# davidbau/rewriting

Measured on AMD Instinct MI355X. Metric: images/sec StyleGANv2-1024 fwd, higher is better.
Workload: dtype f32 (conv operands split into exact f16 pairs from 32x32 up, f32 accumulate); 1 GPU; stylegan2-1024 generator forward (FFHQ-1024 architecture); batch_per_gpu=64, mconv=seq, weights=synthetic seed 0, parallelism=seeds partitioned per rank, no collective, matrix_mode=split, direct_sums=auto

## Files before the change

### include/rewriting_hip.h

```cpp
#ifndef REWRITING_HIP_H
#define REWRITING_HIP_H

#include <stdint.h>

#ifdef __cplusplus
extern "C" {
#endif

typedef void* rw_stream_t;

#define RW_ERR_BAD_ARGUMENT 10001
#define RW_ERR_UNSUPPORTED  10002

int rw_abi_version(void);
const char* rw_error_string(int code);


int rw_fused_bias_act_f32(const float* x, const float* b, const float* ref, float* y,
                          int64_t n, int64_t step_b, int64_t size_b,
                          int act, int grad, float alpha, float scale, rw_stream_t stream);
int rw_fused_bias_act_f16(const uint16_t* x, const uint16_t* b, const uint16_t* ref, uint16_t* y,
                          int64_t n, int64_t step_b, int64_t size_b,
                          int act, int grad, float alpha, float scale, rw_stream_t stream);
int rw_fused_bias_act_f64(const double* x, const double* b, const double* ref, double* y,
// ... 146 lines not shown
                                           const float* post_scale, float u_inv, const float* x_amax,
                                           float* y_amax, rw_stream_t stream);

int rw_dconv3x3_supported(int out_ch, int in_ch, int h, int w);
long long rw_packed_dconv_weight_elems(int out_ch, int in_ch);
int rw_pack_dconv_weight_f32(const float* w, float* wp, int out_ch, int in_ch, float u_scale, rw_stream_t stream);
int rw_dconv3x3_f32(const float* x, const float* wp, float* y, int batch, int in_ch, int out_ch, int h, int w,
                    float w_scale, const rw_conv_epilogue* ep, float u_inv, const float* x_amax, float* y_amax,
                    rw_stream_t stream);
int rw_dconv3x3_rgb_partials(int out_ch);
int rw_dconv3x3_rgb_partial_f32(const float* x, const float* wp, float* y, int batch, int in_ch, int out_ch, int h, int w,
                                float w_scale, const rw_conv_epilogue* ep, const rw_rgb_epilogue* rgb, float u_inv,
                                const float* x_amax, float* y_amax, rw_stream_t stream);
int rw_rgb_combine_f32(const float* partials, int n_part, const float* bias, const float* skip, float* y, int batch,
                       int64_t hw, rw_stream_t stream);
int rw_rgb_combine_up_f32(const float* partials, int n_part, const float* bias, const float* skip_half, const float* k4,
                          float* y, int batch, int h, int w, rw_stream_t stream);
int rw_dconv3x3_to_rgb_supported(int out_ch, int in_ch, int h, int w);
int rw_dconv3x3_to_rgb_f32(const float* x, const float* wp, int batch, int in_ch, int out_ch, int h, int w,
                           float w_scale, const rw_conv_epilogue* ep, const rw_rgb_epilogue* rgb, float u_inv,
                           const float* x_amax, rw_stream_t stream);
int rw_dconv_transpose_blur_supported(int out_ch, int in_ch, int h, int w);
long long rw_packed_dconv_transpose_blur_weight_elems(int out_ch, int in_ch);
int rw_pack_dconv_transpose_blur_weight_f32(const float* w, const float* k4, float* wp, int out_ch, int in_ch,
                                            float u_scale, rw_stream_t stream);
int rw_dconv_transpose3x3s2_blur_f32(const float* x, const float* wp, float* y, int batch, int in_ch, int out_ch, int h,
                                     int w, float w_scale, const rw_conv_epilogue* ep, const float* post_scale,
                                     float u_inv, const float* x_amax, float* y_amax, rw_stream_t stream);

int rw_tconv_blur_supported(int out_ch, int in_ch, int h, int w);
int rw_tconv_blur_f32(const float* x, const float* wp, const float* k4, float* y, int batch, int in_ch, int out_ch, int h,
                      int w, float w_scale, const rw_conv_epilogue* ep, const float* post_scale, float u_inv,
                      const float* x_amax, float* y_amax, rw_stream_t stream);

int rw_conv_transpose3x3s2_winoh_supported(int out_ch, int in_ch, int h, int w);
long long rw_packed_conv_transpose_winoh_elems(int out_ch, int in_ch);
int rw_pack_conv_transpose_winoh_f32(const float* w, float* uf, int out_ch, int in_ch, float u_scale, rw_stream_t stream);
int rw_conv_transpose3x3s2_winoh_f32(const float* x, const float* uf, float* y, int batch, int in_ch, int out_ch,
                                     int h, int w, float w_scale, const float* style, const float* demod, float u_inv,
                                     const float* x_amax, rw_stream_t stream);

int rw_noise_add_f32(const float* x, const float* noise, const float* noise_w, float* y,
                     int batch, int channels, int64_t hw, rw_stream_t stream);

int rw_blur_noise_act_f32(const float* x, const float* k4, const float* noise, const float* noise_w,
                          const float* bias, float* y, int batch, int channels, int out_h, int out_w,
                          rw_stream_t stream);
int rw_blur_noise_act_scaled_f32(const float* x, const float* k4, const float* noise, const float* noise_w,
                                 const float* bias, const float* post_scale, float* y, int batch, int channels,
                                 int out_h, int out_w, rw_stream_t stream);
int rw_blur_noise_act_amax_f32(const float* x, const float* k4, const float* noise, const float* noise_w,
                               const float* bias, const float* post_scale, float* y, int batch, int channels,
                               int out_h, int out_w, float* y_amax, rw_stream_t stream);

int rw_to_rgb_f32(const float* x, const float* w, const float* style, const float* bias,
                  const float* skip, float* y, int batch, int in_ch, int64_t hw, float w_scale,
                  rw_stream_t stream);


int64_t rw_second_moment_workspace_bytes(int channels, int64_t rows);
int rw_second_moment_f32(const float* a, float* mom2, int64_t rows, int channels, int64_t hw,
                         int layout, void* workspace, rw_stream_t stream);

int rw_channel_sums_f32(const float* a, float* sums, int64_t rows, int channels, int64_t hw,
                        int layout, int square_input, rw_stream_t stream);

// ... 153 lines not shown
```

### rewriting_amd/_lib.py

```python
import ctypes
import os
from ctypes import (POINTER, Structure, c_char_p, c_double, c_float, c_int, c_int32, c_int64, c_uint,
                    c_void_p)

_HERE = os.path.dirname(os.path.abspath(__file__))
LIB_PATH = os.environ.get('RW_HIP_LIB') or os.path.join(_HERE, 'librewriting_hip.so')

ABI_VERSION = 11


class ConvEpilogue(Structure):
    _fields_ = [('style', c_void_p), ('demod', c_void_p), ('noise', c_void_p),
                ('noise_w', c_void_p), ('bias', c_void_p), ('act', c_int)]


class RgbEpilogue(Structure):
    _fields_ = [('weight', c_void_p), ('style', c_void_p), ('bias', c_void_p), ('skip', c_void_p),
                ('out', c_void_p), ('scale', c_float)]


LPIPS_MAX_TAPS = 8


class LpipsMaps(Structure):
# ... 121 lines not shown
    'rw_conv_transpose3x3s2_blur_wino4h_f32': (c_int, [c_void_p, c_void_p, c_void_p, c_int, c_int, c_int, c_int,
                                                       c_int, c_float, POINTER(ConvEpilogue), c_void_p, c_float,
                                                       c_void_p, c_void_p, c_void_p]),
    'rw_dconv3x3_supported': (c_int, [c_int, c_int, c_int, c_int]),
    'rw_packed_dconv_weight_elems': (ctypes.c_longlong, [c_int, c_int]),
    'rw_pack_dconv_weight_f32': (c_int, [c_void_p, c_void_p, c_int, c_int, c_float, c_void_p]),
    'rw_dconv3x3_f32': (c_int, [c_void_p, c_void_p, c_void_p, c_int, c_int, c_int, c_int, c_int, c_float,
                                POINTER(ConvEpilogue), c_float, c_void_p, c_void_p, c_void_p]),
    'rw_dconv3x3_rgb_partials': (c_int, [c_int]),
    'rw_dconv3x3_rgb_partial_f32': (c_int, [c_void_p, c_void_p, c_void_p, c_int, c_int, c_int, c_int, c_int, c_float,
                                            POINTER(ConvEpilogue), POINTER(RgbEpilogue), c_float, c_void_p, c_void_p,
                                            c_void_p]),
    'rw_rgb_combine_f32': (c_int, [c_void_p, c_int, c_void_p, c_void_p, c_void_p, c_int, c_int64, c_void_p]),
    'rw_rgb_combine_up_f32': (c_int, [c_void_p, c_int, c_void_p, c_void_p, c_void_p, c_void_p, c_int, c_int, c_int,
                                      c_void_p]),
    'rw_conv3x3_wino4_to_rgb_up_f32': (c_int, [c_void_p, c_void_p, c_int, c_int, c_int, c_int, c_int, c_float,
                                               POINTER(ConvEpilogue), POINTER(RgbEpilogue), c_void_p, c_void_p,
                                               c_void_p]),
    'rw_conv3x3_wino4h_to_rgb_up_f32': (c_int, [c_void_p, c_void_p, c_int, c_int, c_int, c_int, c_int, c_float,
                                                POINTER(ConvEpilogue), POINTER(RgbEpilogue), c_float, c_void_p, c_void_p,
                                                c_void_p, c_void_p]),
    'rw_dconv3x3_to_rgb_supported': (c_int, [c_int, c_int, c_int, c_int]),
    'rw_dconv3x3_to_rgb_f32': (c_int, [c_void_p, c_void_p, c_int, c_int, c_int, c_int, c_int, c_float,
                                       POINTER(ConvEpilogue), POINTER(RgbEpilogue), c_float, c_void_p, c_void_p]),
    'rw_dconv_transpose_blur_supported': (c_int, [c_int, c_int, c_int, c_int]),
    'rw_packed_dconv_transpose_blur_weight_elems': (ctypes.c_longlong, [c_int, c_int]),
    'rw_pack_dconv_transpose_blur_weight_f32': (c_int, [c_void_p, c_void_p, c_void_p, c_int, c_int, c_float, c_void_p]),
    'rw_dconv_transpose3x3s2_blur_f32': (c_int, [c_void_p, c_void_p, c_void_p, c_int, c_int, c_int, c_int, c_int,
                                                 c_float, POINTER(ConvEpilogue), c_void_p, c_float, c_void_p, c_void_p,
                                                 c_void_p]),
    'rw_tconv_blur_supported': (c_int, [c_int, c_int, c_int, c_int]),
    'rw_tconv_blur_f32': (c_int, [c_void_p, c_void_p, c_void_p, c_void_p, c_int, c_int, c_int, c_int, c_int, c_float,
                                  POINTER(ConvEpilogue), c_void_p, c_float, c_void_p, c_void_p, c_void_p]),
    'rw_conv_transpose_blur_wino4_supported': (c_int, [c_int, c_int, c_int, c_int]),
    'rw_packed_conv_transpose_blur_wino4_elems': (ctypes.c_longlong, [c_int, c_int]),
    'rw_pack_conv_transpose_blur_weight_wino4_f32': (c_int, [c_void_p, c_void_p, c_void_p, c_int, c_int, c_void_p]),
    'rw_conv_transpose3x3s2_blur_wino4_f32': (c_int, [c_void_p, c_void_p, c_void_p, c_int, c_int, c_int, c_int,
                                                      c_int, c_float, POINTER(ConvEpilogue), c_void_p, c_void_p]),
    'rw_blur_noise_act_scaled_f32': (c_int, [c_void_p, c_void_p, c_void_p, c_void_p, c_void_p, c_void_p, c_void_p,
                                             c_int, c_int, c_int, c_int, c_void_p]),
    'rw_blur_noise_act_amax_f32': (c_int, [c_void_p, c_void_p, c_void_p, c_void_p, c_void_p, c_void_p, c_void_p,
                                           c_int, c_int, c_int, c_int, c_void_p, c_void_p]),
    'rw_solve_ksplit': (c_int, [c_int, c_int, c_int, c_int]),
    'rw_solve_supported': (c_int, [c_int] * 7),
    'rw_solve_scratch_elems': (c_int, [c_int] * 5 + [POINTER(ctypes.c_longlong)]),
    'rw_solve_step_f32': (c_int, [POINTER(SolveProblem), c_int, c_void_p]),
    'rw_solve_run_supported': (c_int, [c_int] * 7),
    'rw_solve_run_scratch_elems': (ctypes.c_longlong, [c_int] * 5),
    'rw_solve_run_f32': (c_int, [POINTER(SolveProblem), c_int, c_int, c_int, c_int, c_int, c_void_p, c_void_p]),
    'rw_project_weight_f32': (c_int, [c_void_p, c_void_p, c_void_p, c_void_p, c_int, c_int, c_int,
                                      c_int, c_float, c_void_p]),
    'rw_conv_wgrad_ksplit': (c_int, [c_int] * 6),
    'rw_conv_wgrad_f32': (c_int, [c_void_p] * 6 + [c_int] * 6 + [c_float, c_void_p]),
    'rw_rowdot_f32': (c_int, [c_void_p, c_void_p, c_void_p, ctypes.c_longlong, ctypes.c_longlong, c_void_p]),
    'rw_to_rgb_input_grad_f32': (c_int, [c_void_p, c_void_p, c_void_p, c_void_p, c_int, c_int, c_int64, c_float,
                                         c_void_p]),
    'rw_to_rgb_weight_sums_scratch_elems': (ctypes.c_longlong, [c_int, c_int, c_int64]),
    'rw_to_rgb_weight_sums_f32': (c_int, [c_void_p, c_void_p, c_void_p, c_void_p, c_int, c_int, c_int64, c_void_p]),
    'rw_bias_relu_pool_f32': (c_int, [c_void_p, c_void_p, c_void_p, c_void_p, c_int, c_int, c_int, c_int, c_void_p]),
    'rw_bias_relu_pool_grad_f32': (c_int, [c_void_p, c_void_p, c_void_p, c_int, c_int, c_int, c_int, c_int, c_void_p]),
    'rw_conv3x3_rgb_f32': (c_int, [c_void_p, c_void_p, c_void_p, c_void_p, c_int, c_int, c_int, c_int, c_void_p]),
    'rw_conv3x3_rgb_input_grad_f32': (c_int, [c_void_p, c_void_p, c_void_p, c_int, c_int, c_int, c_int, c_void_p]),
    'rw_lpips_tap_f32': (c_int, [c_void_p, c_void_p, c_void_p, c_void_p, c_int, c_int, c_int, c_int64, c_void_p]),
    'rw_lpips_reduce_scratch_elems': (ctypes.c_longlong, [c_int, c_int64]),
    'rw_lpips_combine_f32': (c_int, [POINTER(LpipsMaps), c_void_p, c_void_p, c_void_p, c_int, c_void_p, c_void_p, c_void_p,
                                     c_int, c_int, c_int, c_void_p]),
# ... 58 lines not shown
```

### rewriting_amd/csrc/rw_tconv.hip

```cpp
#include "rw_common.h"
#include <stdio.h>

struct TconvProblem {
  const float* x; const unsigned char* wp; float* y; const float* k4;
  const float* style; const float* demod; const float* noise; const float* noise_w; const float* bias; int act;
  const float* post;
  int batch, in_ch, out_ch, h, w;
  int tiles_x, tiles_y, o_tiles;
  float w_scale, u_inv;
  const float* x_amax; float* y_amax;
};

#define TC_TX 32
#define TC_PC (TC_TX + 2)
#define TC_WC (TC_TX + 3)
#define TC_ZP 72
#define TC_WCH 9216

#ifndef TC_LDS_PAD
#define TC_LDS_PAD 0
#endif
#ifndef TC_ITEM_G
#define TC_ITEM_G 1
#endif
#ifndef TC_AHEAD
#define TC_AHEAD 1
#endif
#ifndef TC_STAGE_PRIO
#define TC_STAGE_PRIO 0
#endif
#ifndef TC_ABL
#define TC_ABL 0
#endif

__device__ __forceinline__ rw_f16x8 tc_pair_hq(rw_f32x2 h, rw_f16x8 q) {
  const rw_f32x4 qq = __builtin_bit_cast(rw_f32x4, q);
  const rw_f32x4 d = {h[0], h[1], qq[0], qq[1]};
  return __builtin_bit_cast(rw_f16x8, d);
}
#ifndef TC_PROF
#define TC_PROF 0
#endif
#if TC_PROF
__device__ unsigned long long tc_prof[64];
extern "C" int rw_tconv_prof(unsigned long long* out) {
  return (int)hipMemcpyFromSymbol(out, HIP_SYMBOL(tc_prof), sizeof(unsigned long long) * 64);
}
#define TP_DECL(...) unsigned long long __VA_ARGS__
#define TP_NOW(t) t = (unsigned long long)clock64()
#define TP_ADD(var, t) { const unsigned long long tp_n = (unsigned long long)clock64(); var += tp_n - t; t = tp_n; }
#else
#define TP_DECL(...)
#define TP_NOW(t)
#define TP_ADD(var, t)
#endif
__device__ __forceinline__ float tc_mul(float a, float b) {
  float r;
  asm("v_mul_f32 %0, %1, %2" : "=v"(r) : "v"(a), "v"(b));
  return r;
}

template <int TY, int WAVES, int NT>
__device__ __forceinline__ void tconv_body(const TconvProblem& p) {
  constexpr int THREADS = 64 * WAVES;
  constexpr int PR = TY + 2;
  constexpr int NPOS = PR * TC_PC, NBLK = (NPOS + 15) / 16, BPW = (NBLK + WAVES - 1) / WAVES;
  constexpr int WR = TY + 3, NPIX = WR * TC_WC;
  constexpr int BUFB = NPIX * 64;
  constexpr int ZR = 2 * PR, CHS = ZR * TC_ZP + 4;
  static_assert(8 * CHS * 4 <= 2 * BUFB, "the z tile of eight channels fits the window buffers");
  constexpr int SR = 2 * TY * 128 / THREADS;
  static_assert(WAVES % 4 == 0 && THREADS % 128 == 0 && SR * (THREADS / 128) == 2 * TY && (SR == 4 || SR == 8),
                "four or eight output rows per strip segment");
  constexpr int OC = 16 * NT, WCH = NT * TC_WCH;
  __shared__ __attribute__((aligned(16))) unsigned char Ls[2 * BUFB];
  __shared__ __attribute__((aligned(16))) unsigned char Wl[2 * WCH];
  __shared__ __attribute__((aligned(16))) float St[512];
  __shared__ float Sc[OC], Bs[OC], Po[OC], Kf[16], Red[WAVES];
#if TC_LDS_PAD
  constexpr int PADB = TY == 16 ? 163840 - 2 * BUFB - 2 * WCH - 2048 - 4 * 64 - 4 * WAVES - 64 : 16;
  __shared__ unsigned char Pad[PADB];
  if (p.batch < 0) Pad[threadIdx.x] = 1;
#endif

  const int tid = threadIdx.x, lane = tid & 63;
  const int wave = __builtin_amdgcn_readfirstlane(tid >> 6);
  const int lk = lane >> 4, lt = lane & 15;

  int ot, tx, ty, ib;
  rw_tile_digits(p, rw_xcd_remap(blockIdx.x, gridDim.x), ot, tx, ty, ib);
  const int I0 = ty * TY, J0 = tx * TC_TX;
  const int64_t hw = (int64_t)p.h * p.w;
  const int NC = p.in_ch >> 4, T = 9 * NC;

  float in_scale, out_scale;
  {
    const float smax = rw_block_max<WAVES>(rw_style_absmax_wave<64 * WAVES>(p, ib, tid), lane, wave, Red);
    rw_split_scales<14>(rw_bound_load(p.x_amax) * smax, p.u_inv, in_scale, out_scale);
  }
  const float gain = p.act ? 1.4142135623730951f : 1.f, slope = p.act ? 0.2f : 1.f;
  for (int i = tid; i < p.in_ch; i += THREADS) St[i] = (p.style ? p.style[(int64_t)ib * p.in_ch + i] : 1.0f) * in_scale;
  if (tid < OC) {
    const int o = OC * ot + tid;
    Sc[tid] = (p.demod ? p.demod[(int64_t)ib * p.out_ch + o] * p.w_scale : p.w_scale) * out_scale * gain;
    Bs[tid] = p.act ? p.bias[o] * gain : 0.f;
    Po[tid] = p.post ? p.post[(int64_t)ib * p.out_ch + o] : 1.f;
  }
  if (tid < 16) {
    const int a = tid >> 2, c = tid & 3;
    Kf[tid] = p.k4[(3 - a) * 4 + (3 - c)];
  }
  const float noise_wg = p.noise ? p.noise_w[0] * gain : 0.f;
  __syncthreads();

  constexpr int NSL = WAVES / 4;
  const int g = wave & 3, hsel = wave >> 2;
  const __amdgpu_buffer_rsrc_t xsrc = rw_image_rsrc(p.x, ib, p.in_ch, hw);
  const int hw4 = (int)hw * 4;
  constexpr int IPR = TC_TX / 4 + 2, NITEM = WR * IPR;
  constexpr int SI = (NITEM + 64 * NSL - 1) / (64 * NSL), LPP = ((NITEM + SI * NSL - 1) / (SI * NSL) + 3) & ~3;
  static_assert(SI <= 2 && LPP <= 64 && LPP * SI * NSL >= NITEM, "one or two pieces per wave cover the window");
  int xoff[SI], lofa[SI], lofb[SI], lok[SI];
#pragma unroll
  for (int s = 0; s < SI; ++s) {
    const int li = TC_ITEM_G == 4 ? (lane & 3) * (LPP / 4) + (lane >> 2) : lane;
    const int it = LPP * (NSL * s + hsel) + li;
    const bool mine = lane < LPP && it < NITEM;
    const int r = it / IPR, j = it - r * IPR;
    const int iy = I0 - 2 + r, ix = J0 - 4 + 4 * j;
    const bool ok = mine && iy >= 0 && iy < p.h && ix >= 0 && ix < p.w;
    xoff[s] = ok ? (iy * p.w + ix) * 4 : 0x7ffffff0;
    const int cc0 = 4 * j - 2;
    lofa[s] = (r * TC_WC + cc0) * 64 + ((g ^ rw_swz(cc0 & 0x7ffffffe)) << 4);
    lofb[s] = (r * TC_WC + cc0 + 2) * 64 + ((g ^ rw_swz(cc0 + 2)) << 4);
// ... 14 lines not shown
  };
  auto stage_store_part = [&](int c, int buf, auto s_tag, auto e0_tag, auto e1_tag) __attribute__((always_inline)) {
    constexpr int s = decltype(s_tag)::value, E0 = decltype(e0_tag)::value, E1 = decltype(e1_tag)::value;
    const rw_f32x4 sv = *reinterpret_cast<const rw_f32x4*>(&St[16 * c + 4 * g]);
    unsigned char* dst = Ls + buf * BUFB;
#pragma unroll
    for (int e = E0; e < E1; ++e) {
      const float v0 = tc_mul(raw[s][0][e], sv[0]), v1 = tc_mul(raw[s][1][e], sv[1]), v2 = tc_mul(raw[s][2][e], sv[2]),
                  v3 = tc_mul(raw[s][3][e], sv[3]);
      rw_f16x8 word = rw_split4(v0, v1, v2, v3);
      if (TC_ABL & 256)
        word = __builtin_bit_cast(rw_f16x8, rw_f32x4{raw[s][0][e], raw[s][1][e], raw[s][2][e], raw[s][3][e]});
      if (TC_ABL & 512) { asm volatile("" :: "v"(word)); }
      else if (lok[s] & (1 << e)) *reinterpret_cast<rw_f16x8*>(dst + (e < 2 ? lofa[s] : lofb[s]) + (e & 1) * 64) = word;
    }
  };
  const unsigned char* wsrc = p.wp + (int64_t)(NT * ot) * T * 1024;
  constexpr int NPC = NT * (TC_WCH / 16), NWP = (NPC + THREADS - 1) / THREADS;
  rw_f32x4 wraw[NWP];
  auto wstage_load = [&](int c) __attribute__((always_inline)) {
#pragma unroll
    for (int k = 0; k < NWP; ++k) {
      const int pc = tid + k * THREADS < NPC ? tid + k * THREADS : NPC - 1;
      const int n = pc / (TC_WCH / 16), r = pc - n * (TC_WCH / 16);
      wraw[k] = *reinterpret_cast<const rw_f32x4*>(wsrc + ((int64_t)n * T + 9 * c) * 1024 + r * 16);
    }
  };
  auto wstage_store = [&](int buf) __attribute__((always_inline)) {
    unsigned char* dst = Wl + buf * WCH;
#pragma unroll
    for (int k = 0; k < NWP; ++k)
      if ((k + 1) * THREADS <= NPC || tid + k * THREADS < NPC)
        *reinterpret_cast<rw_f32x4*>(dst + (tid + k * THREADS) * 16) = wraw[k];
  };

  unsigned pb0[BPW], pb1[BPW];
#pragma unroll
  for (int b = 0; b < BPW; ++b) {
    int q = 16 * (wave + WAVES * b) + lt;
    q = q < NPOS ? q : NPOS - 1;
    const int r = q / TC_PC, c = q - r * TC_PC;
    pb0[b] = (unsigned)((r * TC_WC + c + 1) * 64 + ((lk ^ rw_swz(c + 1)) << 4));
    pb1[b] = (unsigned)((r * TC_WC + c) * 64 + ((lk ^ rw_swz(c)) << 4));
  }

  rw_f32x4 acc[BPW][NT][4];
#pragma unroll
  for (int b = 0; b < BPW; ++b)
#pragma unroll
    for (int n = 0; n < NT; ++n)
#pragma unroll
      for (int ph = 0; ph < 4; ++ph) acc[b][n][ph] = rw_f32x4{0.f, 0.f, 0.f, 0.f};

#define TB_MFMA(PH, A, B) acc[b][n][PH] = __builtin_amdgcn_mfma_f32_16x16x32_f16(A, B, acc[b][n][PH], 0, 0, 0)
#define TB_UH(T_) rw_expand(*reinterpret_cast<const rw_f32x2*>(wb + n * TC_WCH + (T_) * 1024))
#define TB_UL(T_) (*reinterpret_cast<const rw_f32x2*>(wb + n * TC_WCH + (T_) * 1024 + 512))
#define TC_PIX(OFF) (*reinterpret_cast<const rw_f16x8*>(lb + (OFF)))
#define TC_VH(OFF) (*reinterpret_cast<const rw_f32x2*>(lb + (OFF)))
#define TC_MFMA(PH, A, B) acc[b][PH] = __builtin_amdgcn_mfma_f32_16x16x32_f16(A, B, acc[b][PH], 0, 0, 0)
#define TC_UH(T_) rw_expand(*reinterpret_cast<const rw_f32x2*>(wb + (T_) * 1024))
#define TC_UL(T_) (*reinterpret_cast<const rw_f32x2*>(wb + (T_) * 1024 + 512))
  TP_DECL(tp = 0, tp_all = 0, tp_g0 = 0, tp_s0 = 0, tp_g1 = 0, tp_g2 = 0, tp_s1 = 0, tp_bar = 0, tp_pro = 0);
  auto chunk = [&](int c, auto last_tag) __attribute__((always_inline)) {
    constexpr bool LAST = decltype(last_tag)::value != 0;
    const int buf = c & 1;
    const unsigned char* lb = Ls;
    const unsigned char* wb = Wl + buf * WCH + lane * 8;
    TP_NOW(tp);
    constexpr bool st = !LAST;
    const int c2 = c + 2 < NC ? c + 2 : NC - 1;
    auto hook = [&](auto grp_tag, int b) __attribute__((always_inline)) {
      constexpr int grp = decltype(grp_tag)::value;
#if TC_PROF
      if (b < 4) { if (grp == 0) { TP_ADD(tp_g0, tp); } else if (grp == 1) { TP_ADD(tp_g1, tp); } else { TP_ADD(tp_g2, tp); } }
#endif
      if constexpr (grp < SI) {
        if (b == 0 && st) stage_store_part(c + 1, buf ^ 1, rw_int<grp>(), rw_int<0>(), rw_int<2>());
        if (b == 1 && st) stage_store_part(c + 1, buf ^ 1, rw_int<grp>(), rw_int<2>(), rw_int<4>());
        if constexpr (BPW >= 4) {
          if (b == 2) stage_load_part(c2, rw_int<grp>(), rw_int<0>(), rw_int<2>());
          if (b == 3) stage_load_part(c2, rw_int<grp>(), rw_int<2>(), rw_int<4>());
        } else {
          if (b == 2) stage_load_part(c2, rw_int<grp>(), rw_int<0>(), rw_int<4>());
        }
      } else if constexpr (grp == 2) {
        if (b == 0 && st) wstage_store(buf ^ 1);
        if (b == 1) wstage_load(c2);
      }
#if TC_PROF
      if (b < 2) { TP_ADD(tp_s0, tp); } else if (b < 4) { TP_ADD(tp_s1, tp); }
#endif
    };
    constexpr int LB = BPW - 1;
    const bool last_ok = wave + WAVES * LB < NBLK;
    {
      rw_f16x8 u0[NT], u1[NT], u3[NT], u4[NT], l4[NT];
#pragma unroll
      for (int n = 0; n < NT; ++n) { u0[n] = TB_UH(0); u1[n] = TB_UH(1); u3[n] = TB_UH(3); u4[n] = TB_UH(4); l4[n] = rw_expand(TB_UL(4)); }
      rw_f16x8 pc = TC_PIX(pb0[0] + TC_WC * 64), pd = pc;
      if (TC_AHEAD == 2 && BPW > 1) pd = TC_PIX(pb0[1] + TC_WC * 64);
#pragma unroll
      for (int b = 0; b < BPW; ++b) {
        rw_f16x8 pn = TC_AHEAD == 2 ? pd : pc;
        if (b + TC_AHEAD < BPW) pn = TC_PIX(pb0[b + TC_AHEAD] + TC_WC * 64);
        if (b < LB || last_ok) {
#pragma unroll
          for (int n = 0; n < NT; ++n) {
            if (TC_ABL & 2) { asm volatile("" :: "v"(pc), "v"(u0[n]), "v"(u1[n]), "v"(u3[n]), "v"(u4[n]), "v"(l4[n])); }
            else {
// ... 45 lines not shown
        u6[n] = TB_UH(6); u7[n] = TB_UH(7); u8[n] = TB_UH(8);
        m17[n] = rw_pair(TB_UL(1), TB_UL(7)); m68[n] = rw_pair(TB_UL(6), TB_UL(8));
      }
      rw_f32x2 hc = TC_VH(pb0[0] + TC_WC * 64), hd = hc;
      rw_f16x8 qc = TC_PIX(pb0[0]), rc = TC_PIX(pb1[0]), qd = qc, rd = rc;
      if (TC_AHEAD == 2 && BPW > 1) { hd = TC_VH(pb0[1] + TC_WC * 64); qd = TC_PIX(pb0[1]); rd = TC_PIX(pb1[1]); }
#pragma unroll
      for (int b = 0; b < BPW; ++b) {
        rw_f32x2 hn = TC_AHEAD == 2 ? hd : hc;
        rw_f16x8 qn = TC_AHEAD == 2 ? qd : qc, rn = TC_AHEAD == 2 ? rd : rc;
        if (b + TC_AHEAD < BPW) { hn = TC_VH(pb0[b + TC_AHEAD] + TC_WC * 64); qn = TC_PIX(pb0[b + TC_AHEAD]); rn = TC_PIX(pb1[b + TC_AHEAD]); }
        if (b < LB || last_ok) {
          const rw_f16x8 M02 = tc_pair_hq(hc, qc), M23 = rw_pair(qc, rc);
#pragma unroll
          for (int n = 0; n < NT; ++n) {
            if (TC_ABL & 2) { asm volatile("" :: "v"(hc), "v"(qc), "v"(rc), "v"(u6[n]), "v"(u7[n]), "v"(u8[n]), "v"(m17[n]), "v"(m68[n])); }
            else {
              TB_MFMA(0, qc, u6[n]); TB_MFMA(1, qc, u7[n]);
              TB_MFMA(0, rc, u8[n]); TB_MFMA(1, M02, m17[n]);
              TB_MFMA(0, M23, m68[n]);
            }
          }
        }
        hook(rw_int<2>(), b);
        __builtin_amdgcn_sched_barrier(0);
        if (TC_AHEAD == 2) { hc = hd; qc = qd; rc = rd; hd = hn; qd = qn; rd = rn; } else { hc = hn; qc = qn; rc = rn; }
      }
    }
    TP_ADD(tp_g2, tp);
    if (!LAST) {
      const unsigned delta = buf ? (unsigned)-BUFB : (unsigned)BUFB;
#pragma unroll
      for (int b = 0; b < BPW; ++b) { pb0[b] += delta; pb1[b] += delta; }
      asm volatile("" ::: "memory");
      __builtin_amdgcn_s_waitcnt(0xC07F);
      __builtin_amdgcn_s_barrier();
      asm volatile("" ::: "memory");
      TP_ADD(tp_bar, tp);
    }
  };

  TP_NOW(tp_all);
  wstage_load(0);
#pragma unroll
  for (int s = 0; s < SI; ++s) {
    if (s == 0) stage_load_part(0, rw_int<0>(), rw_int<0>(), rw_int<4>());
    else stage_load_part(0, rw_int<SI - 1>(), rw_int<0>(), rw_int<4>());
  }
  stage_store_part(0, 0, rw_int<0>(), rw_int<0>(), rw_int<4>());
  if constexpr (SI > 1) stage_store_part(0, 0, rw_int<SI - 1>(), rw_int<0>(), rw_int<4>());
  wstage_store(0);
  __syncthreads();
  {
    const int c1 = NC > 1 ? 1 : 0;
    __builtin_amdgcn_sched_barrier(0);
    stage_load_part(c1, rw_int<0>(), rw_int<0>(), rw_int<4>());
    __builtin_amdgcn_sched_barrier(0);
    if constexpr (SI > 1) stage_load_part(c1, rw_int<SI - 1>(), rw_int<0>(), rw_int<4>());
    __builtin_amdgcn_sched_barrier(0);
    wstage_load(c1);
    __builtin_amdgcn_sched_barrier(0);
  }

#if TC_PROF
  TP_NOW(tp); tp_pro = tp - tp_all;
#endif
  for (int c = 0; c + 1 < NC; ++c) chunk(c, rw_int<0>());
  chunk(NC - 1, rw_int<1>());
#if TC_PROF
  const unsigned long long tp_loop_end = (unsigned long long)clock64();
#endif
  if (TC_ABL & 8) { if (acc[0][0][0][0] != 12345.f) return; }
  __syncthreads();

  float* Z = reinterpret_cast<float*>(Ls);
  float ymax = 0.f;
  float kf[16];
#pragma unroll
  for (int t = 0; t < 16; ++t) kf[t] = Kf[t];
  bool sep = kf[0] != 0.f;
  float kv[4], kmax = 0.f;
#pragma unroll
  for (int t = 0; t < 16; ++t) kmax = fmaxf(kmax, fabsf(kf[t]));
#pragma unroll
  for (int a = 0; a < 4; ++a) kv[a] = sep ? kf[4 * a] / kf[0] : 0.f;
#pragma unroll
  for (int t = 0; t < 16; ++t) sep = sep && fabsf(kf[t] - kv[t >> 2] * kf[t & 3]) <= 1e-6f * kmax;
  const int W2 = 2 * p.w;
  const int64_t hw2 = 4 * hw;
  const int strip = tid & 127, seg = tid >> 7;
  const int s_og = strip & 15, s_ch = strip >> 4, s_oy0 = SR * seg;
  const int64_t s_pix = (int64_t)(2 * I0 + s_oy0) * W2 + 2 * J0 + 4 * s_og;
  rw_f32x4 nzr[SR];
#pragma unroll
  for (int oy = 0; oy < SR; ++oy) {
// ... 86 lines not shown
        }
        const int cl = 16 * n + 8 * pass + ch;
        const int64_t pix = (int64_t)(2 * I0 + oy) * W2 + 2 * J0 + 4 * og;
        rw_f32x4 nz = {0.f, 0.f, 0.f, 0.f};
        if (p.noise) nz = *reinterpret_cast<const rw_f32x4*>(p.noise + (int64_t)ib * hw2 + pix) * noise_wg;
        const float sc = Sc[cl], bs = Bs[cl], post = Po[cl];
        rw_f32x4 v;
#pragma unroll
        for (int q = 0; q < 4; ++q) {
          const float u = res[q] * sc + nz[q] + bs;
          v[q] = fmaxf(u, u * slope) * post;
          ymax = fmaxf(ymax, fabsf(v[q]));
        }
        *reinterpret_cast<rw_f32x4*>(p.y + ((int64_t)ib * p.out_ch + OC * ot + cl) * hw2 + pix) = v;
      }
    }
    __syncthreads();
  }
  }
#if TC_PROF
  if (lane == 0 && (wave == 0 || wave == 7) && (blockIdx.x == gridDim.x / 2 || blockIdx.x == gridDim.x / 2 + 777)) {
    unsigned long long* o = tc_prof + (blockIdx.x == gridDim.x / 2 ? 0 : 32) + (wave == 0 ? 0 : 16);
    const unsigned long long now = (unsigned long long)clock64();
    o[0] = now - tp_all; o[1] = tp_pro; o[2] = tp_g0; o[3] = tp_s0; o[4] = tp_g1; o[5] = tp_g2; o[6] = tp_s1; o[7] = tp_bar;
    o[8] = now - tp_loop_end; o[9] = NC;
  }
#endif
  if (p.y_amax) rw_bound_store_wave(p.y_amax, rw_wave_max(ymax));
}

__global__ void __launch_bounds__(256, 2) tconv_blur_t8_kernel(const TconvProblem p) { tconv_body<8, 4, 1>(p); }
__global__ void __launch_bounds__(512, 1) tconv_blur_t16_kernel(const TconvProblem p) { tconv_body<16, 8, 1>(p); }
__global__ void __launch_bounds__(512, 1) tconv_blur_n32_kernel(const TconvProblem p) { tconv_body<8, 8, 2>(p); }

#ifndef TC_NT
#define TC_NT 0
#endif
#ifndef TC_PP_MQ
#define TC_PP_MQ 2
#endif

template <int MW>
__device__ __forceinline__ void tconv_ws_body(const TconvProblem& p) {
  constexpr int TY = 8;
  constexpr int PR = TY + 2, NPOS = PR * TC_PC, NBLK = (NPOS + 15) / 16, BPW = (NBLK + MW - 1) / MW;
  constexpr int WR = TY + 3, NPIX = WR * TC_WC, BUFB = NPIX * 64;
  constexpr int IPR = TC_TX / 4 + 2, NITEM = WR * IPR, SI = (NITEM + 63) / 64;
  constexpr int ZR = 2 * PR + 2, CHS = ZR * TC_ZP + 4;
  constexpr int SR = 4, CT = 512;
  static_assert(SI == 2 && BPW == 24 / MW && (MW == 4 || MW == 8) && SR * (CT / 128) == 2 * TY, "piece / block / strip counts the code below is written for");
  constexpr bool STAGERS_BLUR = MW == 4;
  __shared__ __attribute__((aligned(16))) unsigned char Ls[2 * BUFB];
  __shared__ __attribute__((aligned(16))) unsigned char Wl[2 * TC_WCH];
  __shared__ __attribute__((aligned(16))) float Zs[8 * CHS];
  __shared__ float Sc[2][16], Bs[2][16], Po[2][16], Kf[16], Ks[12];

  const int tid = threadIdx.x, lane = tid & 63;
  const int wave = __builtin_amdgcn_readfirstlane(tid >> 6);
  const int64_t hw = (int64_t)p.h * p.w;
  const int NC = p.in_ch >> 4, T = 9 * NC;
  const float gain = p.act ? 1.4142135623730951f : 1.f, slope = p.act ? 0.2f : 1.f;

  const int64_t total = (int64_t)p.batch * p.tiles_y * p.tiles_x * p.o_tiles;
  const int bx = rw_xcd_remap(blockIdx.x, gridDim.x);
  const int count = (int)((total - bx + gridDim.x - 1) / gridDim.x);
  if (count <= 0) {
    if (p.y_amax) rw_bound_store_wave(p.y_amax, 0.f);
// ... 870 lines not shown
  for (int n = 0; n < N; ++n) {
    const unsigned char* lb = Ls + (n & 1) * BUFB;
    const unsigned char* wb = Wl + (n & 1) * TC_WCH + lane * 8;
    mma(lb, wb);
    TP_ADD(tp_mma, tp);
    rw_lds_barrier();
    TP_ADD(tp_bar, tp);
    if (c + 1 < NC) { ++c; continue; }
    c = 0;
    if (TC_PP_MQ > 0) noise_request(ty, tx, ib);
    zwrite();
    TP_ADD(tp_zw, tp);
    rw_lds_barrier();
    TP_ADD(tp_zbar, tp);
#pragma unroll 1
    for (int ps = 0; ps < TC_PP_MQ; ++ps) blur(ps, pos & 3, ot, tx, ty, ib);
    TP_ADD(tp_blur, tp);
    ++pos;
    walk.advance(ot, tx, ty, ib);
#pragma unroll
    for (int b = 0; b < BPW; ++b)
#pragma unroll
      for (int ph = 0; ph < 4; ++ph) acc[b][ph] = rw_f32x4{0.f, 0.f, 0.f, 0.f};
  }
#if TC_PROF
  if (wave == 0 && lane == 0 && (blockIdx.x == 0 || blockIdx.x == 100)) {
    unsigned long long* o = tc_prof + (blockIdx.x == 0 ? 0 : 32);
    o[0] = (unsigned long long)clock64() - tp_all; o[1] = tp_mma; o[2] = tp_bar; o[3] = tp_zw; o[4] = tp_blur; o[5] = tp_zbar; o[6] = N;
  }
#endif
  if (p.y_amax) rw_bound_store_wave(p.y_amax, rw_wave_max(ymax));
}

static bool tconv_shape_ok(int out_ch, int in_ch, int h, int w) {
  return out_ch > 0 && out_ch % 16 == 0 && in_ch >= 16 && in_ch % 16 == 0 && in_ch <= 512 && w % TC_TX == 0 && h % 16 == 0;
}

extern "C" int rw_tconv_blur_supported(int out_ch, int in_ch, int h, int w) { return tconv_shape_ok(out_ch, in_ch, h, w) ? 1 : 0; }

extern "C" int rw_tconv_blur_f32(const float* x, const float* wp, const float* k4, float* y, int batch, int in_ch,
                                 int out_ch, int h, int w, float w_scale, const rw_conv_epilogue* ep,
                                 const float* post_scale, float u_inv, const float* x_amax, float* y_amax,
                                 rw_stream_t stream) {
  RW_CHECK_ARG(x && wp && k4 && y && x_amax && u_inv > 0.f && batch > 0 && in_ch > 0 && out_ch > 0 && h > 0 && w > 0);
  RW_CHECK_ARG(rw_epilogue_ok(ep));
  if (!tconv_shape_ok(out_ch, in_ch, h, w)) return RW_ERR_UNSUPPORTED;
  if ((int64_t)in_ch * h * w * 4 > 0x7fffffffLL) return RW_ERR_UNSUPPORTED;
  TconvProblem p = {};
  p.x = x; p.wp = reinterpret_cast<const unsigned char*>(wp); p.y = y; p.k4 = k4;
  rw_fill_epilogue(p, ep);
  p.post = post_scale;
  p.batch = batch; p.in_ch = in_ch; p.out_ch = out_ch; p.h = h; p.w = w; p.w_scale = w_scale; p.u_inv = u_inv;
  p.x_amax = x_amax; p.y_amax = y_amax;
  const int persistent = rw_env_int("RW_TCONV_PERSISTENT", 0) == 2 ? 2 : 0;
  int n32_lo = 1, n32_hi = 0;
  if (const char* ne = getenv("RW_TCONV_N32")) { if (sscanf(ne, "%d:%d", &n32_lo, &n32_hi) != 2) { n32_lo = 1; n32_hi = 0; } }
  const int sel = rw_env_int("RW_TCONV_TY", out_ch % 32 == 0 && in_ch >= n32_lo && in_ch <= n32_hi ? 32
                                           : (in_ch >= 32 && in_ch <= 128 ? persistent : 16));
  if ((sel == 0 || sel == 2 || sel == 12) && in_ch >= 32) {
    p.tiles_x = w / TC_TX; p.tiles_y = h / 8; p.o_tiles = out_ch / 16;
    const int64_t tiles = (int64_t)batch * p.tiles_y * p.tiles_x * p.o_tiles;
    if (tiles <= 0 || tiles > 0x7fffffff) return RW_ERR_UNSUPPORTED;
    int64_t grid = rw_env_int("RW_TCONV_GRID", rw_cu_count());
    grid = grid < 1 ? 1 : (grid > tiles ? tiles : grid);
    const int wv = sel == 12 ? 12 : 8;
    if (y_amax && wv * grid > rw_bound_slot_capacity((int64_t)batch * out_ch * 4 * h * w)) return RW_ERR_UNSUPPORTED;
    if (sel == 2) hipLaunchKernelGGL(tconv_blur_pp_kernel, dim3((unsigned)grid), dim3(512), 0, rw_s(stream), p);
    else if (sel == 12) hipLaunchKernelGGL(tconv_blur_ws12_kernel, dim3((unsigned)grid), dim3(768), 0, rw_s(stream), p);
    else hipLaunchKernelGGL(tconv_blur_ws_kernel, dim3((unsigned)grid), dim3(512), 0, rw_s(stream), p);
    return rw_finish_bound(y_amax, wv * grid, stream);
  }
  const bool n32 = sel == 32 && out_ch % 32 == 0;
  const int ty = sel == 16 ? 16 : 8;
  const int waves = ty == 16 || n32 ? 8 : 4;
  p.tiles_x = w / TC_TX; p.tiles_y = h / ty; p.o_tiles = out_ch / (n32 ? 32 : 16);
  const int64_t work = (int64_t)batch * p.tiles_y * p.tiles_x * p.o_tiles;
  if (work <= 0 || work > 0x7fffffff) return RW_ERR_UNSUPPORTED;
  if (y_amax && waves * work > rw_bound_slot_capacity((int64_t)batch * out_ch * 4 * h * w)) return RW_ERR_UNSUPPORTED;
  if (n32) hipLaunchKernelGGL(tconv_blur_n32_kernel, dim3((unsigned)work), dim3(512), 0, rw_s(stream), p);
  else if (ty == 16) hipLaunchKernelGGL(tconv_blur_t16_kernel, dim3((unsigned)work), dim3(512), 0, rw_s(stream), p);
  else hipLaunchKernelGGL(tconv_blur_t8_kernel, dim3((unsigned)work), dim3(256), 0, rw_s(stream), p);
  return rw_finish_bound(y_amax, waves * work, stream);
}
```

### rewriting_amd/hip.py

```python
import ctypes
from collections import namedtuple as _namedtuple

import torch

from . import _lib
from ._lib import ConvEpilogue, RgbEpilogue, SolveProblem, check

SQRT2 = 2 ** 0.5


def _stream():
    return ctypes.c_void_p(torch.cuda.current_stream().cuda_stream)


def _dev(t, name='tensor', dtype=torch.float32):
    if not isinstance(t, torch.Tensor):
        raise TypeError('%s must be a torch.Tensor' % name)
    if not t.is_cuda:
        raise RuntimeError('rewriting_amd: %s is on %s; the HIP kernels need a GPU tensor '
                           '(there is no CPU fallback)' % (name, t.device))
    if t.dtype != dtype:
        if dtype == torch.float32:
            raise RuntimeError('rewriting_amd: %s is %s; the C ABI is fp32 only (RW_ERR_UNSUPPORTED, include/rewriting_hip.h: '
                               'the reference\'s pybind modules also dispatch half and double, this library does not) -- '
# ... 693 lines not shown
    _conv('rw_dconv3x3_rgb_partial_f32', x, _packed(wp, out_ch, x.shape[1], _DIRECT16), out_ch, w_scale,
          _epilogue(style, demod, noise, noise_w, bias, act), x_amax=x_amax, y=y, y_amax=y_amax,
          rgb=_rgb_epilogue(rgb_weight, rgb_style, None, None, rgb_scale, part, x, out_ch))
    return y, part


def conv3x3_direct16_to_rgb(x, wp, out_ch, w_scale, rgb_weight, rgb_style, rgb_bias, rgb_skip, rgb_scale, style=None,
                            demod=None, noise=None, noise_w=None, bias=None, act=False, x_amax=None):
    x = _dev(x, 'fmap')
    rgb = _out(x, 3)
    _conv('rw_dconv3x3_to_rgb_f32', x, _packed(wp, out_ch, x.shape[1], _DIRECT16), out_ch, w_scale,
          _epilogue(style, demod, noise, noise_w, bias, act), x_amax=x_amax,
          rgb=_rgb_epilogue(rgb_weight, rgb_style, rgb_bias, rgb_skip, rgb_scale, rgb, x, out_ch))
    return None, rgb


def conv_transpose3x3s2_blur_direct16(x, wp, out_ch, w_scale, style=None, demod=None, noise=None, noise_w=None,
                                      bias=None, act=False, post_scale=None, x_amax=None, y_amax=None):
    x = _dev(x, 'fmap')
    y = _out(x, out_ch, up=2)
    _conv('rw_dconv_transpose3x3s2_blur_f32', x, _packed(wp, out_ch, x.shape[1], _UP_BLUR_DIRECT16), out_ch, w_scale,
          _epilogue(style, demod, noise, noise_w, bias, act), x_amax=x_amax, y=y,
          post_scale=_post_scale(post_scale, x.shape[0], out_ch), y_amax=y_amax)
    return y


tconv_blur_supported = _supported('rw_tconv_blur_supported', 'Shapes conv_transpose3x3s2_blur_fused takes')


def conv_transpose3x3s2_blur_fused(x, wp, k4, out_ch, w_scale, style=None, demod=None, noise=None, noise_w=None,
                                   bias=None, act=False, post_scale=None, x_amax=None, y_amax=None):
    x = _dev(x, 'fmap')
    y = _out(x, out_ch, up=2)
    _conv('rw_tconv_blur_f32', x, _packed(wp, out_ch, x.shape[1], _DIRECT16), out_ch, w_scale,
          _epilogue(style, demod, noise, noise_w, bias, act), x_amax=x_amax, k4=_k4(k4), y=y,
          post_scale=_post_scale(post_scale, x.shape[0], out_ch), y_amax=y_amax)
    return y


_workspaces = {}


def _workspace(nbytes, device):
    key = (device.index, torch.cuda.current_stream(device).cuda_stream)
    ws = _workspaces.get(key)
    if ws is None or ws.numel() < nbytes:
        ws = torch.empty(max(nbytes, 1 << 20), dtype=torch.uint8, device=device)
        _workspaces[key] = ws
    return ws


def second_moment_accumulate(mom2, a, nchw=False):
    a = _dev(a, 'sample')
    if not (mom2.is_cuda and mom2.dtype == torch.float32 and mom2.is_contiguous()):
        raise RuntimeError('mom2 must be a contiguous float32 GPU tensor')
    if nchw:
        b, c, h, w = a.shape
        rows, hw, layout = b * h * w, h * w, 1
        if hw % 16:
            a = a.permute(0, 2, 3, 1).reshape(-1, c).contiguous()
            rows, hw, layout = a.shape[0], 0, 0
    else:
        rows, c = a.shape
        hw, layout = 0, 0
    if mom2.shape != (c, c):
        raise RuntimeError('mom2 is %s, the sample has %d channels' % (tuple(mom2.shape), c))
    out = mom2
    if layout == 0 and c % 4:
        a = torch.nn.functional.pad(a, (0, 4 - c % 4))
# ... 544 lines not shown
```

Before: 1635 images/sec.

## Pre-split tconv input into f16 pair words and DMA-stage them directly into LDS

For transposed-conv-blur layers with at least 256 input channels, a separate split_map kernel first converts the modulated f32 input into f16 split words in a workspace buffer. A staged variant of the tconv kernel then copies both weights and these prepared words straight into LDS with buffer/global DMA requests, replacing the in-kernel load, style-multiply, split and LDS-store path. The aim is to take register and VALU work off the main loop and overlap the copies with compute. In exchange it adds an extra kernel launch, a full-size intermediate write and read, and host-side buffer registration. The path is skipped during graph capture.

```diff
diff --git a/include/rewriting_hip.h b/include/rewriting_hip.h
--- a/include/rewriting_hip.h
+++ b/include/rewriting_hip.h
@@ -202,6 +202,8 @@
 int rw_tconv_blur_f32(const float* x, const float* wp, const float* k4, float* y, int batch, int in_ch, int out_ch, int h,
                       int w, float w_scale, const rw_conv_epilogue* ep, const float* post_scale, float u_inv,
                       const float* x_amax, float* y_amax, rw_stream_t stream);
+long long rw_tconv_stage_bytes(int batch, int in_ch, int out_ch, int h, int w);
+int rw_tconv_stage_buffer(rw_stream_t stream, void* ptr, long long bytes);
 
 int rw_conv_transpose3x3s2_winoh_supported(int out_ch, int in_ch, int h, int w);
 long long rw_packed_conv_transpose_winoh_elems(int out_ch, int in_ch);
diff --git a/rewriting_amd/_lib.py b/rewriting_amd/_lib.py
--- a/rewriting_amd/_lib.py
+++ b/rewriting_amd/_lib.py
@@ -177,6 +177,8 @@
     'rw_tconv_blur_supported': (c_int, [c_int, c_int, c_int, c_int]),
     'rw_tconv_blur_f32': (c_int, [c_void_p, c_void_p, c_void_p, c_void_p, c_int, c_int, c_int, c_int, c_int, c_float,
                                   POINTER(ConvEpilogue), c_void_p, c_float, c_void_p, c_void_p, c_void_p]),
+    'rw_tconv_stage_bytes': (ctypes.c_longlong, [c_int, c_int, c_int, c_int, c_int]),
+    'rw_tconv_stage_buffer': (c_int, [c_void_p, c_void_p, ctypes.c_longlong]),
     'rw_conv_transpose_blur_wino4_supported': (c_int, [c_int, c_int, c_int, c_int]),
     'rw_packed_conv_transpose_blur_wino4_elems': (ctypes.c_longlong, [c_int, c_int]),
     'rw_pack_conv_transpose_blur_weight_wino4_f32': (c_int, [c_void_p, c_void_p, c_void_p, c_int, c_int, c_void_p]),
diff --git a/rewriting_amd/csrc/rw_tconv.hip b/rewriting_amd/csrc/rw_tconv.hip
--- a/rewriting_amd/csrc/rw_tconv.hip
+++ b/rewriting_amd/csrc/rw_tconv.hip
@@ -1,5 +1,6 @@
 #include "rw_common.h"
 #include <stdio.h>
+#include <mutex>
 
 struct TconvProblem {
   const float* x; const unsigned char* wp; float* y; const float* k4;
@@ -60,7 +61,7 @@
   return r;
 }
 
-template <int TY, int WAVES, int NT>
+template <int TY, int WAVES, int NT, bool STAGED = false>
 __device__ __forceinline__ void tconv_body(const TconvProblem& p) {
   constexpr int THREADS = 64 * WAVES;
   constexpr int PR = TY + 2;
@@ -99,7 +100,8 @@
     rw_split_scales<14>(rw_bound_load(p.x_amax) * smax, p.u_inv, in_scale, out_scale);
   }
   const float gain = p.act ? 1.4142135623730951f : 1.f, slope = p.act ? 0.2f : 1.f;
-  for (int i = tid; i < p.in_ch; i += THREADS) St[i] = (p.style ? p.style[(int64_t)ib * p.in_ch + i] : 1.0f) * in_scale;
+  if constexpr (!STAGED)
+    for (int i = tid; i < p.in_ch; i += THREADS) St[i] = (p.style ? p.style[(int64_t)ib * p.in_ch + i] : 1.0f) * in_scale;
   if (tid < OC) {
     const int o = OC * ot + tid;
     Sc[tid] = (p.demod ? p.demod[(int64_t)ib * p.out_ch + o] * p.w_scale : p.w_scale) * out_scale * gain;
@@ -180,6 +182,47 @@
     for (int k = 0; k < NWP; ++k)
       if ((k + 1) * THREADS <= NPC || tid + k * THREADS < NPC)
         *reinterpret_cast<rw_f32x4*>(dst + (tid + k * THREADS) * 16) = wraw[k];
+  };
+
+  constexpr int NSLOT = NPIX * 4, NPC_S = (NSLOT + 63) / 64, PPW = (NPC_S + WAVES - 1) / WAVES;
+  constexpr int NWPC = 9 * NT, NWS = (NWPC + WAVES - 1) / WAVES;
+  static_assert(NSLOT >= 64 && NWS + PPW <= 3 * BPW, "one request behind each position block of a chunk");
+  typedef __attribute__((address_space(3))) unsigned char* lds_b;
+  const unsigned ls_base = (unsigned)(size_t)(lds_b)Ls, wl_base = (unsigned)(size_t)(lds_b)Wl;
+  const unsigned long long xw_addr = (unsigned long long)(p.x + (int64_t)ib * p.in_ch * hw);
+  const rw_i32x4 xsrc_w = {(int)(unsigned)xw_addr, (int)(unsigned)(xw_addr >> 32), (int)((int64_t)p.in_ch * hw * 4), 0x00020000};
+  int voff[PPW], sslot[PPW];
+  if constexpr (STAGED) {
+#pragma unroll
+    for (int k = 0; k < PPW; ++k) {
+      const int first = 64 * (wave + WAVES * k);
+      sslot[k] = first < NSLOT - 64 ? first : NSLOT - 64;
+      const int L = sslot[k] + lane, pix = L >> 2, s = L & 3;
+      const int r = pix / TC_WC, c = pix - r * TC_WC;
+      const int iy = I0 - 2 + r, ix = J0 - 2 + c;
+      const bool ok = iy >= 0 && iy < p.h && ix >= 0 && ix < p.w;
+      voff[k] = ok ? (iy * p.w + ix) * 64 + ((s ^ rw_swz(c)) << 4) : 0x7ffffff0;
+    }
+  }
+  auto copy_request = [&](int c, int buf, int q) __attribute__((always_inline)) {
+#pragma unroll
+    for (int k = 0; k < NWS; ++k)
+      if (q == k) {
+        const int first = wave + WAVES * k, wpc = first < NWPC ? first : NWPC - 1;
+        const int n = wpc / 9, r = wpc - 9 * n;
+        rw_dma_global_b128_s(wl_base + (unsigned)(buf * WCH + wpc * 1024), lane * 16,
+                             wsrc + ((int64_t)n * T + 9 * c) * 1024 + r * 1024);
+      }
+#pragma unroll
+    for (int k = 0; k < PPW; ++k)
+      if (q == NWS + k)
+        rw_dma_buffer_b128(ls_base + (unsigned)(buf * BUFB + sslot[k] * 16), voff[k], xsrc_w, c * hw4 * 16);
+  };
+  auto copy_wait = [&]() __attribute__((always_inline)) {
+    asm volatile("" ::: "memory");
+    __builtin_amdgcn_s_waitcnt(0x0070);
+    __builtin_amdgcn_s_barrier();
+    asm volatile("" ::: "memory");
   };
 
   unsigned pb0[BPW], pb1[BPW];
@@ -222,7 +265,9 @@
 #if TC_PROF
       if (b < 4) { if (grp == 0) { TP_ADD(tp_g0, tp); } else if (grp == 1) { TP_ADD(tp_g1, tp); } else { TP_ADD(tp_g2, tp); } }
 #endif
-      if constexpr (grp < SI) {
+      if constexpr (STAGED) {
+        if (st) copy_request(c + 1, buf ^ 1, grp * BPW + b);
+      } else if constexpr (grp < SI) {
         if (b == 0 && st) stage_store_part(c + 1, buf ^ 1, rw_int<grp>(), rw_int<0>(), rw_int<2>());
         if (b == 1 && st) stage_store_part(c + 1, buf ^ 1, rw_int<grp>(), rw_int<2>(), rw_int<4>());
         if constexpr (BPW >= 4) {
@@ -334,15 +379,23 @@
       const unsigned delta = buf ? (unsigned)-BUFB : (unsigned)BUFB;
 #pragma unroll
       for (int b = 0; b < BPW; ++b) { pb0[b] += delta; pb1[b] += delta; }
-      asm volatile("" ::: "memory");
-      __builtin_amdgcn_s_waitcnt(0xC07F);
-      __builtin_amdgcn_s_barrier();
-      asm volatile("" ::: "memory");
+      if constexpr (STAGED) copy_wait();
+      else {
+        asm volatile("" ::: "memory");
+        __builtin_amdgcn_s_waitcnt(0xC07F);
+        __builtin_amdgcn_s_barrier();
+        asm volatile("" ::: "memory");
+      }
       TP_ADD(tp_bar, tp);
     }
   };
 
   TP_NOW(tp_all);
+  if constexpr (STAGED) {
+#pragma unroll
+    for (int q = 0; q < NWS + PPW; ++q) copy_request(0, 0, q);
+    copy_wait();
+  } else {
   wstage_load(0);
 #pragma unroll
   for (int s = 0; s < SI; ++s) {
@@ -363,6 +416,7 @@
     wstage_load(c1);
     __builtin_amdgcn_sched_barrier(0);
   }
+  }
 
 #if TC_PROF
   TP_NOW(tp); tp_pro = tp - tp_all;
@@ -515,7 +569,6 @@
 __global__ void __launch_bounds__(256, 2) tconv_blur_t8_kernel(const TconvProblem p) { tconv_body<8, 4, 1>(p); }
 __global__ void __launch_bounds__(512, 1) tconv_blur_t16_kernel(const TconvProblem p) { tconv_body<16, 8, 1>(p); }
 __global__ void __launch_bounds__(512, 1) tconv_blur_n32_kernel(const TconvProblem p) { tconv_body<8, 8, 2>(p); }
-
 #ifndef TC_NT
 #define TC_NT 0
 #endif
@@ -1452,11 +1505,106 @@
   if (p.y_amax) rw_bound_store_wave(p.y_amax, rw_wave_max(ymax));
 }
 
+__global__ void __launch_bounds__(256, 2) tconv_blur_t8s_kernel(const TconvProblem p) { tconv_body<8, 4, 1, true>(p); }
+__global__ void __launch_bounds__(512, 1) tconv_blur_t16s_kernel(const TconvProblem p) { tconv_body<16, 8, 1, true>(p); }
+__global__ void __launch_bounds__(512, 1) tconv_blur_n32s_kernel(const TconvProblem p) { tconv_body<8, 8, 2, true>(p); }
+
+struct SplitMapProblem {
+  const float* x; unsigned char* words; const float* style; const float* x_amax;
+  int batch, in_ch, h, w, iters;
+  float u_inv;
+};
+__global__ void __launch_bounds__(256) split_map_kernel(const SplitMapProblem p) {
+  __shared__ float Red[4];
+  const int tid = threadIdx.x, lane = tid & 63;
+  const int wave = __builtin_amdgcn_readfirstlane(tid >> 6);
+  const int ib = blockIdx.z, ch = blockIdx.y;
+  float in_scale, out_scale;
+  {
+    const float smax = rw_block_max<4>(rw_style_absmax_wave<256>(p, ib, tid), lane, wave, Red);
+    rw_split_scales<14>(rw_bound_load(p.x_amax) * smax, p.u_inv, in_scale, out_scale);
+  }
+  const int g = tid & 3, c0 = 16 * ch + 4 * g;
+  float sv[4];
+#pragma unroll
+  for (int k = 0; k < 4; ++k) sv[k] = (p.style ? p.style[(int64_t)ib * p.in_ch + c0 + k] : 1.0f) * in_scale;
+  const int64_t hw = (int64_t)p.h * p.w;
+  const float* xi = p.x + ((int64_t)ib * p.in_ch + c0) * hw;
+  unsigned char* wo = p.words + ((int64_t)ib * p.in_ch + 16 * ch) * hw * 4 + g * 16;
+  for (int it = 0; it < p.iters; ++it) {
+    const int64_t pix = 4 * (((int64_t)blockIdx.x * p.iters + it) * 64 + (tid >> 2));
+    rw_f32x4 raw[4];
+#pragma unroll
+    for (int k = 0; k < 4; ++k) raw[k] = *reinterpret_cast<const rw_f32x4*>(xi + k * hw + pix);
+#pragma unroll
+    for (int e = 0; e < 4; ++e)
+      *reinterpret_cast<rw_f16x8*>(wo + (pix + e) * 64) =
+          rw_split4(tc_mul(raw[0][e], sv[0]), tc_mul(raw[1][e], sv[1]), tc_mul(raw[2][e], sv[2]), tc_mul(raw[3][e], sv[3]));
+  }
+}
+
 static bool tconv_shape_ok(int out_ch, int in_ch, int h, int w) {
   return out_ch > 0 && out_ch % 16 == 0 && in_ch >= 16 && in_ch % 16 == 0 && in_ch <= 512 && w % TC_TX == 0 && h % 16 == 0;
 }
 
 extern "C" int rw_tconv_blur_supported(int out_ch, int in_ch, int h, int w) { return tconv_shape_ok(out_ch, in_ch, h, w) ? 1 : 0; }
+
+#ifndef RW_TCONV_STAGED_DEFAULT
+#define RW_TCONV_STAGED_DEFAULT 1
+#endif
+#ifndef RW_TCONV_STAGED_MIN_IN_DEFAULT
+#define RW_TCONV_STAGED_MIN_IN_DEFAULT 256
+#endif
+static int tconv_form(int in_ch, int out_ch) {
+  const int persistent = rw_env_int("RW_TCONV_PERSISTENT", 0) == 2 ? 2 : 0;
+  int n32_lo = 1, n32_hi = 0;
+  if (const char* ne = getenv("RW_TCONV_N32")) { if (sscanf(ne, "%d:%d", &n32_lo, &n32_hi) != 2) { n32_lo = 1; n32_hi = 0; } }
+  const int sel = rw_env_int("RW_TCONV_TY", out_ch % 32 == 0 && in_ch >= n32_lo && in_ch <= n32_hi ? 32
+                                           : (in_ch >= 32 && in_ch <= 128 ? persistent : 16));
+  return sel;
+}
+static bool tconv_staged_wanted(int sel, int in_ch, int batch) {
+  if ((sel == 0 || sel == 2 || sel == 12) && in_ch >= 32) return false;
+  return rw_env_int("RW_TCONV_STAGED", RW_TCONV_STAGED_DEFAULT) != 0 &&
+         in_ch >= rw_env_int("RW_TCONV_STAGED_MIN_IN", RW_TCONV_STAGED_MIN_IN_DEFAULT) && batch <= 65535;
+}
+namespace {
+struct StageBuffer { int dev; hipStream_t stream; void* ptr; long long bytes; };
+constexpr int kStageBuffers = 64;
+StageBuffer g_stage[kStageBuffers];
+std::mutex g_stage_lock;
+}
+extern "C" long long rw_tconv_stage_bytes(int batch, int in_ch, int out_ch, int h, int w) {
+  if (batch <= 0 || !tconv_shape_ok(out_ch, in_ch, h, w) || (int64_t)in_ch * h * w * 4 > 0x7fffffffLL) return 0;
+  if (!tconv_staged_wanted(tconv_form(in_ch, out_ch), in_ch, batch)) return 0;
+  return (long long)batch * in_ch * h * w * 4;
+}
+extern "C" int rw_tconv_stage_buffer(rw_stream_t stream, void* ptr, long long bytes) {
+  RW_CHECK_ARG((ptr == nullptr) == (bytes == 0) && bytes >= 0 && (reinterpret_cast<uintptr_t>(ptr) & 15) == 0);
+  int dev = 0;
+  if (hipGetDevice(&dev) != hipSuccess) return RW_ERR_UNSUPPORTED;
+  std::lock_guard<std::mutex> hold(g_stage_lock);
+  StageBuffer* slot = nullptr;
+  for (StageBuffer& b : g_stage)
+    if (b.ptr && b.dev == dev && b.stream == rw_s(stream)) slot = &b;
+  if (!ptr) {
+    if (slot) *slot = StageBuffer{};
+    return 0;
+  }
+  for (StageBuffer& b : g_stage)
+    if (!slot && !b.ptr) slot = &b;
+  if (!slot) return RW_ERR_UNSUPPORTED;
+  *slot = StageBuffer{dev, rw_s(stream), ptr, bytes};
+  return 0;
+}
+static void* tconv_stage_lookup(rw_stream_t stream, long long need) {
+  int dev = 0;
+  if (hipGetDevice(&dev) != hipSuccess) return nullptr;
+  std::lock_guard<std::mutex> hold(g_stage_lock);
+  for (const StageBuffer& b : g_stage)
+    if (b.ptr && b.dev == dev && b.stream == rw_s(stream)) return b.bytes >= need ? b.ptr : nullptr;
+  return nullptr;
+}
 
 extern "C" int rw_tconv_blur_f32(const float* x, const float* wp, const float* k4, float* y, int batch, int in_ch,
                                  int out_ch, int h, int w, float w_scale, const rw_conv_epilogue* ep,
@@ -1472,11 +1620,7 @@
   p.post = post_scale;
   p.batch = batch; p.in_ch = in_ch; p.out_ch = out_ch; p.h = h; p.w = w; p.w_scale = w_scale; p.u_inv = u_inv;
   p.x_amax = x_amax; p.y_amax = y_amax;
-  const int persistent = rw_env_int("RW_TCONV_PERSISTENT", 0) == 2 ? 2 : 0;
-  int n32_lo = 1, n32_hi = 0;
-  if (const char* ne = getenv("RW_TCONV_N32")) { if (sscanf(ne, "%d:%d", &n32_lo, &n32_hi) != 2) { n32_lo = 1; n32_hi = 0; } }
-  const int sel = rw_env_int("RW_TCONV_TY", out_ch % 32 == 0 && in_ch >= n32_lo && in_ch <= n32_hi ? 32
-                                           : (in_ch >= 32 && in_ch <= 128 ? persistent : 16));
+  const int sel = tconv_form(in_ch, out_ch);
   if ((sel == 0 || sel == 2 || sel == 12) && in_ch >= 32) {
     p.tiles_x = w / TC_TX; p.tiles_y = h / 8; p.o_tiles = out_ch / 16;
     const int64_t tiles = (int64_t)batch * p.tiles_y * p.tiles_x * p.o_tiles;
@@ -1497,6 +1641,22 @@
   const int64_t work = (int64_t)batch * p.tiles_y * p.tiles_x * p.o_tiles;
   if (work <= 0 || work > 0x7fffffff) return RW_ERR_UNSUPPORTED;
   if (y_amax && waves * work > rw_bound_slot_capacity((int64_t)batch * out_ch * 4 * h * w)) return RW_ERR_UNSUPPORTED;
+  void* words = nullptr;
+  if (tconv_staged_wanted(sel, in_ch, batch)) words = tconv_stage_lookup(stream, (long long)batch * in_ch * h * w * 4);
+  if (words) {
+    SplitMapProblem sp = {};
+    sp.x = x; sp.words = static_cast<unsigned char*>(words); sp.style = p.style; sp.x_amax = x_amax;
+    sp.batch = batch; sp.in_ch = in_ch; sp.h = h; sp.w = w; sp.u_inv = u_inv;
+    const int blocks = h * w / 256;
+    sp.iters = blocks % 4 == 0 ? 4 : 2;
+    hipLaunchKernelGGL(split_map_kernel, dim3((unsigned)(blocks / sp.iters), (unsigned)(in_ch / 16), (unsigned)batch), dim3(256),
+                       0, rw_s(stream), sp);
+    p.x = reinterpret_cast<const float*>(sp.words);
+    if (n32) hipLaunchKernelGGL(tconv_blur_n32s_kernel, dim3((unsigned)work), dim3(512), 0, rw_s(stream), p);
+    else if (ty == 16) hipLaunchKernelGGL(tconv_blur_t16s_kernel, dim3((unsigned)work), dim3(512), 0, rw_s(stream), p);
+    else hipLaunchKernelGGL(tconv_blur_t8s_kernel, dim3((unsigned)work), dim3(256), 0, rw_s(stream), p);
+    return rw_finish_bound(y_amax, waves * work, stream);
+  }
   if (n32) hipLaunchKernelGGL(tconv_blur_n32_kernel, dim3((unsigned)work), dim3(512), 0, rw_s(stream), p);
   else if (ty == 16) hipLaunchKernelGGL(tconv_blur_t16_kernel, dim3((unsigned)work), dim3(512), 0, rw_s(stream), p);
   else hipLaunchKernelGGL(tconv_blur_t8_kernel, dim3((unsigned)work), dim3(256), 0, rw_s(stream), p);
diff --git a/rewriting_amd/hip.py b/rewriting_amd/hip.py
--- a/rewriting_amd/hip.py
+++ b/rewriting_amd/hip.py
@@ -749,9 +749,18 @@
                                    bias=None, act=False, post_scale=None, x_amax=None, y_amax=None):
     x = _dev(x, 'fmap')
     y = _out(x, out_ch, up=2)
-    _conv('rw_tconv_blur_f32', x, _packed(wp, out_ch, x.shape[1], _DIRECT16), out_ch, w_scale,
-          _epilogue(style, demod, noise, noise_w, bias, act), x_amax=x_amax, k4=_k4(k4), y=y,
-          post_scale=_post_scale(post_scale, x.shape[0], out_ch), y_amax=y_amax)
+    nbytes = lib().rw_tconv_stage_bytes(x.shape[0], x.shape[1], out_ch, x.shape[2], x.shape[3])
+    staged = nbytes > 0 and not torch.cuda.is_current_stream_capturing()
+    if staged:
+        ws = _workspace(nbytes, x.device)
+        check(lib().rw_tconv_stage_buffer(_stream(), _p(ws), ws.numel()))
+    try:
+        _conv('rw_tconv_blur_f32', x, _packed(wp, out_ch, x.shape[1], _DIRECT16), out_ch, w_scale,
+              _epilogue(style, demod, noise, noise_w, bias, act), x_amax=x_amax, k4=_k4(k4), y=y,
+              post_scale=_post_scale(post_scale, x.shape[0], out_ch), y_amax=y_amax)
+    finally:
+        if staged:
+            check(lib().rw_tconv_stage_buffer(_stream(), None, 0))
     return y
 
 
```

Measured after the change: 1674 images/sec, median of 6. 1.02x the previous value.
